# vniclas/VFM-Registration

Hardware: AMD Instinct MI355X
Metric: registrations/sec (20k<->200k pts, 384-D) (higher is better)
Workload: dtype fp6 (MX e2m3) coarse pass (scaled MFMA, fp32 scores + bounds from measured residuals) + int8 rescan (exact integer scores) + f32 refinement + f64 exact decision / f64 RANSAC

## Files before the change

### vfm-registration_amd/csrc/config.cpp

```cpp
#include "common.h"
#include "config.h"

#include <string.h>

#include <new>

struct vfm_config {
    VfmConfig c;
};

static const VfmConfig k_factory{};
static thread_local const VfmConfig* t_bound = nullptr;

const VfmConfig& vfm_cfg() { return t_bound ? *t_bound : k_factory; }

namespace {
struct Field {
    const char* name;
    int VfmConfig::*p;
};
const Field k_fields[] = {
    {"coarse_slices", &VfmConfig::force_slices},     {"match_stats", &VfmConfig::match_stats},
    {"i8_min_queries", &VfmConfig::i8_min_queries},  {"prep_grid", &VfmConfig::prep_grid},
    {"ransac_exact_only", &VfmConfig::ransac_exact_only}, {"ransac_fused", &VfmConfig::ransac_fused},
    {"coarse_qsets", &VfmConfig::coarse_qsets},      {"seed_units", &VfmConfig::seed_units},
    {"select_variant", &VfmConfig::select_variant},  {"mx6_t4", &VfmConfig::mx6_t4},
    {"mx6_tune", &VfmConfig::mx6_tune},
    {"mx6_ns3", &VfmConfig::mx6_ns3},                {"prep_form", &VfmConfig::prep_form},
    {"finish_short", &VfmConfig::finish_short},      {"rescan_rows", &VfmConfig::rescan_rows},
    {"half_noi8", &VfmConfig::half_noi8},            {"rescore_block", &VfmConfig::rescore_block},
    {"vit_preprocess_patch", &VfmConfig::vit_preprocess_patch}, {"vit_xcd", &VfmConfig::vit_xcd},
    {"vit_cfg_narrow", &VfmConfig::vit_cfg_narrow},  {"vit_cfg_wide", &VfmConfig::vit_cfg_wide},
    {"vit_wpw", &VfmConfig::vit_wpw},                {"vit_hot_a", &VfmConfig::vit_hot_a},
    {"vit_wide_tile", &VfmConfig::vit_wide_tile},    {"vit_lds_shape", &VfmConfig::vit_lds_shape},
    {"vit_att_lds_min", &VfmConfig::vit_att_lds_min}, {"vit_lds_min_wg", &VfmConfig::vit_lds_min_wg},
    {"vit_astat_min", &VfmConfig::vit_astat_min},    {"vit_astat_two", &VfmConfig::vit_astat_two},
    {"vit_astat_nw", &VfmConfig::vit_astat_nw},      {"vit_fused_qkv", &VfmConfig::vit_fused_qkv},
    {"vit_trace_fused", &VfmConfig::vit_trace_fused},  {"vit_fused_mlp", &VfmConfig::vit_fused_mlp},
    {"voxel_replay2", &VfmConfig::voxel_replay2},    {"voxel_one_launch", &VfmConfig::voxel_small},
    {"voxel_trace", &VfmConfig::voxel_trace},        {"voxel_grid_ppt", &VfmConfig::voxel_grid_ppt},
};

const char* const k_trace_buffer = "vit_trace_buffer";

void set_coarse_variant(VfmConfig& c, int v) {
    if (v == 60 || v == 61) { c.rescan_rows = v == 61 ? 1 : 0; return; }
    if (v == 50 || v == 51) { c.finish_short = v == 51 ? 1 : 0; return; }
    if (v >= 40 && v <= 44) { c.prep_form = v == 44 ? 4 : v == 43 ? 3 : v == 41 ? 1 : 0; return; }
    if (v == 32 || v == 33) { c.mx6_ns3 = v == 33 ? 1 : 0; return; }
    if (v == 30 || v == 31) { c.mx6_t4 = v == 30 ? 1 : 0; return; }
    c.seed_units = v == 7 ? 0 : 1;
    if (v == 7) v = 0;
    c.select_variant = v == 20 ? 1 : (v == 21 ? 2 : 0);
    if (v == 20 || v == 21) v = 0;
    c.coarse_qsets = v;
}
void set_voxel_small(VfmConfig& c, int on) {
    if (on == 2 || on == 3) c.voxel_replay2 = on == 3;
    else if (on >= 10 && on <= 10 + 64) c.voxel_grid_ppt = on - 10;
    else if (on == 100 || on == 101) c.voxel_trace = on - 100;
    else c.voxel_small = on;
}
}

VFM_EXPORT int vfm_config_create(vfm_config_t** out) {
    VFM_CHECK_ARG(out, "config_create: null pointer");
    *out = new (std::nothrow) vfm_config();
    if (!*out) return vfm_fail(VFM_EINVAL, "config_create: out of memory");
    return VFM_OK;
}
VFM_EXPORT int vfm_config_destroy(vfm_config_t* cfg) {
    if (cfg && t_bound == &cfg->c) t_bound = nullptr;
    delete cfg;
    return VFM_OK;
}
VFM_EXPORT int vfm_config_use(const vfm_config_t* cfg) {
    t_bound = cfg ? &cfg->c : nullptr;
    return VFM_OK;
}
VFM_EXPORT int vfm_config_set(vfm_config_t* cfg, const char* key, int64_t value) {
    VFM_CHECK_ARG(cfg && key, "config_set: null pointer");
    if ((!strcmp(key, "coarse_variant") && value == 42) || (!strcmp(key, "prep_form") && value == 2))
        return vfm_fail(VFM_EINVAL, "config_set: %s %lld (fp6 operand preparation by width) has been removed", key, (long long)value);
    if (!strcmp(key, "rescore_block") && value != 64 && value != 256)
        return vfm_fail(VFM_EINVAL, "config_set: rescore_block %lld (a workgroup of match_rescore_kernel owns 64 or 256 queries)", (long long)value);
    if (!strcmp(key, "coarse_variant")) { set_coarse_variant(cfg->c, (int)value); return VFM_OK; }
    if (!strcmp(key, "voxel_small")) { set_voxel_small(cfg->c, (int)value); return VFM_OK; }
    if (!strcmp(key, k_trace_buffer)) { cfg->c.vit_astat_dbg = reinterpret_cast<unsigned long long*>((uintptr_t)value); return VFM_OK; }
    for (const Field& f : k_fields)
        if (!strcmp(key, f.name)) {
            cfg->c.*(f.p) = (int)value;
            return VFM_OK;
        }
    return vfm_fail(VFM_EINVAL, "config_set: unknown key '%s'", key);
}
VFM_EXPORT int vfm_config_get(const vfm_config_t* cfg, const char* key, int64_t* value) {
    VFM_CHECK_ARG(key && value, "config_get: null pointer");
    const VfmConfig& c = cfg ? cfg->c : vfm_cfg();
    if (!strcmp(key, k_trace_buffer)) { *value = (int64_t)(uintptr_t)c.vit_astat_dbg; return VFM_OK; }
    for (const Field& f : k_fields)
        if (!strcmp(key, f.name)) {
            *value = c.*(f.p);
            return VFM_OK;
        }
    return vfm_fail(VFM_EINVAL, "config_get: unknown key '%s'", key);
}
```

### vfm-registration_amd/csrc/config.h

```cpp
#pragma once

struct VfmConfig {
    int force_slices = 0;
    int coarse_qsets = 0;
    int seed_units = 1;
    int select_variant = 0;
    int mx6_t4 = 1;
    int mx6_ns3 = 1;
    int prep_form = 3;
    int finish_short = 0;
    int half_noi8 = 1;
    int rescore_block = 0;
    int rescan_rows = 1;
    int mx6_tune = 0;
    int match_stats = 0;
    int i8_min_queries = 0;
    int prep_grid = -1;
    int ransac_exact_only = 0;
    int ransac_fused = 2;
    int vit_preprocess_patch = 1, vit_xcd = 1, vit_cfg_narrow = 108, vit_cfg_wide = 108, vit_wpw = 0, vit_hot_a = 0, vit_wide_tile = 0,
        vit_lds_shape = 23, vit_att_lds_min = 1, vit_lds_min_wg = 256, vit_astat_min = 0, vit_astat_two = 1, vit_astat_nw = 0,
        vit_trace_fused = 0,
        vit_fused_mlp = 0,
        vit_fused_qkv = 0;
    unsigned long long* vit_astat_dbg = nullptr;
    int voxel_replay2 = 1, voxel_small = 1, voxel_trace = 0, voxel_grid_ppt = 0;
};

const VfmConfig& vfm_cfg();
```

### vfm-registration_amd/csrc/match_internal.h

```cpp
#pragma once
#include "common.h"
#include "../../include/vfmreg_debug.h"

#include <type_traits>
#include <vector>

typedef _Float16 half8 __attribute__((ext_vector_type(8)));
typedef _Float16 half4 __attribute__((ext_vector_type(4)));
typedef float floatx16 __attribute__((ext_vector_type(16)));
typedef int intx4 __attribute__((ext_vector_type(4)));
typedef int intx8 __attribute__((ext_vector_type(8)));
typedef int intx16 __attribute__((ext_vector_type(16)));

#define GLOBAL_AS __attribute__((address_space(1)))
#define LDS_AS __attribute__((address_space(3)))

namespace vfmm {

constexpr int TILE_ROWS = 32;
constexpr int CHUNK_ROWS = 128;
constexpr int ROW_PAD = 256;
constexpr int QBLOCK = 256;
constexpr int ring_depth(int ksteps) { return ksteps <= 24 ? 6 : 4; }
constexpr int CAND_CAP_MAX = 2048;
// ... 681 lines not shown
        l.nqb = q2 ? (nq_tiles + 15) / 16 : npad / QBLOCK;
        l.nslices = choose_slices(l.nqb, nchunks);
        if (q2) inst = coarse_inst(CF_I8Q2, p.half ? d / 64 : d / 32, top2, !p.half, p.fused);
        else if (p.half) inst = coarse_inst(CF_I8, d / 64, 4, false, false);
        else inst = coarse_inst(CF_I8, d / 32, d <= 384 && (top2 || !t2) ? 4 : 2, top2, true);
    } else {
        const bool half = p.half, fuse = p.fused;
        const bool ns3 = half && fuse && d == 384 && cfg.mx6_ns3 && cfg.mx6_t4;
        l.nqb = ns3 ? (nq_tiles + 23) / 24 : (nq_tiles + 15) / 16;
        l.nslices = choose_slices(l.nqb, nchunks);
        if (half && cfg.force_slices == 0) {
            int s = (int)((1600 + l.nqb - 1) / l.nqb);
            const int smax = nchunks / 8 < 64 ? nchunks / 8 : 64;
            s = s > smax ? smax : s;
            s = s < 1 ? 1 : s;
            {
                const int cus = compute_units;
                int best = s;
                double best_fill = 0.0;
                for (int t = (s + 4 < smax ? s + 4 : smax); t >= 1 && t >= s - 12; --t) {
                    const long long wg = (long long)l.nqb * t, rounds = (wg + cus - 1) / cus;
                    const double fill = (double)wg / (double)(rounds * cus);
                    if (fill >= 0.975) {
                        best = t;
                        best_fill = 2.0;
                        break;
                    }
                    if (fill > best_fill) {
                        best_fill = fill;
                        best = t;
                    }
                }
                s = best;
            }
            l.nslices = s < 1 ? 1 : s;
        }
        while ((nchunks + l.nslices - 1) / l.nslices + 1 > MX6_LTAB && l.nslices < nchunks) ++l.nslices;
        if (fuse && (l.nqb > surv_slot_qblocks(npad) || l.nslices > surv_slot_slices(nchunks)))
            return vfm_fail(VFM_EINVAL, "search_coarse: %d x %d survivor slots exceed the workspace (n %d chunks %d)", l.nqb, l.nslices, npad, nchunks);
        const bool t8 = half && fuse && (d == 384 || d == 256) && !cfg.mx6_t4 && l.nslices <= nchunks / 2;
        l.tune = cfg.mx6_tune;
        const int ring = ns3 ? ((cfg.mx6_tune & 2) ? 5 : 4) : t8 ? 3 : 4;
        inst = coarse_inst(CF_MX6, half ? d / 128 : d / 64, fuse ? MX6_FUSE : top2 ? MX6_TOP2 : MX6_BEST, !half && !fuse, d / 64, ring, t8 ? 8 : 4, ns3 ? 3 : 2);
    }
    if (inst < 0) return vfm_fail(VFM_EINVAL, "search_coarse: no coarse kernel for d = %d, record kind %d", d, p.kind);
    l.inst = inst;
    l.seeded = l.nseed_pad != 0;
    l.block = coarse_inst_block(k_coarse_insts[inst]);
    l.lds = coarse_inst_lds(k_coarse_insts[inst]);
    return VFM_OK;
}
inline I8Bounds i8_bounds(const Prepared& Q, const Prepared& B, bool on, int top2 = 0) {
    return on ? I8Bounds{Q.err, Q.gstep, B.gstep, B.gerr, top2 == VFM_RECORDS_TOP2 ? 1 : 0} : I8Bounds{nullptr, nullptr, nullptr, nullptr, 0};
}
inline I8Bounds mx6_bounds(const Prepared& Q, const Prepared& B, int top2 = 0) { return I8Bounds{Q.err6, Q.gstep6, B.gstep6, B.gerr6, top2}; }
inline I8Bounds mx6_bounds_half(const Prepared& Q, const Prepared& B) { return I8Bounds{Q.err6h, Q.gstep6, B.gstep6, B.gerr6h, 0}; }
inline I8Bounds plan_bounds(const SearchPlan& p, const Prepared& Q, const Prepared& B) {
    if (p.bounds == BOUNDS_MX6_HALF) return mx6_bounds_half(Q, B);
    if (p.bounds == BOUNDS_MX6) return mx6_bounds(Q, B, p.top2 ? 1 : 0);
    return i8_bounds(Q, B, p.bounds == BOUNDS_I8, p.top2 ? 1 : 0);
}
CoarseArgs coarse_args(const Prepared& Q, const Prepared& B, const SearchWs& w, int64_t n, int64_t m);

struct PrepZero {
    uint4* a = nullptr;
    size_t na = 0;
    uint4* b = nullptr;
    size_t nb = 0;
};
inline PrepZero prep_zero(void* ws, int64_t n, int64_t m) {
    const SearchWs w = carve_search(ws, n, m);
    PrepZero z;
    z.a = reinterpret_cast<uint4*>(w.fb_count);
    z.na = search_zero_bytes(n, m) / 16;
    z.b = reinterpret_cast<uint4*>(w.cand_cnt);
    z.nb = (size_t)rows_padded(n) * sizeof(int) / 16;
    return z;
}
enum PrepInst : unsigned char {
    PREP_ROWS, PREP_CHUNK_BOTH, PREP_CHUNK_2, PREP_CHUNK_3, PREP_CHUNK_MX6,
    PREP_STREAM,
    PREP_ONCE = PREP_STREAM + 4,
    PREP_ONCE_NOI8 = PREP_ONCE + 8,
    PREP_MX6_ROWS_16 = PREP_ONCE_NOI8 + 4, PREP_MX6_ROWS_32, PREP_MX6_GROUP, PREP_INST_COUNT
};
inline const char* prep_inst_name(int inst) {
    static const char* const names[PREP_INST_COUNT] = {
        "prep_rows_kernel", "prep_chunk_kernel<true,2>", "prep_chunk_kernel<false,2>", "prep_chunk_kernel<false,3>", "prep_chunk_kernel<false,2,true,8>",
        "prep_stream_kernel<256,full>", "prep_stream_kernel<256,half>", "prep_stream_kernel<384,full>", "prep_stream_kernel<384,half>",
        "prep_once_kernel<256,full,short>", "prep_once_kernel<256,full,persist>", "prep_once_kernel<256,half,short>", "prep_once_kernel<256,half,persist>",
        "prep_once_kernel<384,full,short>", "prep_once_kernel<384,full,persist>", "prep_once_kernel<384,half,short>", "prep_once_kernel<384,half,persist>",
        "prep_once_kernel<256,half,short,noi8>", "prep_once_kernel<256,half,persist,noi8>", "prep_once_kernel<384,half,short,noi8>",
        "prep_once_kernel<384,half,persist,noi8>", "prep_mx6_rows_kernel<16>", "prep_mx6_rows_kernel<32>", "prep_mx6_group_kernel"};
    return names[inst];
}
enum PrepGridRule : unsigned char { PREP_GRID_ROWS, PREP_GRID_CU, PREP_GRID_2CU_STREAM, PREP_GRID_N };
enum PrepZeroAt : unsigned char { PREP_ZERO_NONE, PREP_ZERO_INSIDE, PREP_ZERO_BEHIND };
struct PrepLaunch {
    int inst;
    bool half6;
    int block, lds;
    int rule, n;
};
struct PrepPlan {
    bool f16 = false, i8 = false, fp6 = false, fp6_half = false;
    PrepLaunch launches[4] = {};
    int nlaunches = 0;
    int zero = PREP_ZERO_NONE;
};

inline int resolve_prepare(PrepPlan& p, int entry, int schedule, int d, int64_t rows1, int dtype1, int64_t rows2, int dtype2, bool zero) {
    p = PrepPlan{};
    const bool single = entry == VFM_PREP_ENTRY_PREPARE || entry == VFM_PREP_ENTRY_PERM;
    const bool gated = entry >= VFM_PREP_ENTRY_GATED && entry <= VFM_PREP_ENTRY_GATED_T;
    const bool scheduled = entry >= VFM_PREP_ENTRY_GATED_P && entry <= VFM_PREP_ENTRY_GATED_T;
    if (entry < VFM_PREP_ENTRY_PREPARE || entry > VFM_PREP_ENTRY_ONESHOT) return vfm_fail(VFM_EINVAL, "prepare: unknown entry %d", entry);
    if (!(rows1 > 0 && (single ? rows2 == 0 : rows2 > 0) && d % 128 == 0 && d >= 128 && d <= 768))
        return vfm_fail(VFM_EINVAL, "%s: d must be in {128,256,384,512,640,768}", entry == VFM_PREP_ENTRY_PREPARE ? "prepare" : "prepare2");
    if (entry == VFM_PREP_ENTRY_PERM && !i8_capable(d)) return vfm_fail(VFM_EINVAL, "prepare(perm): no int8 image for d = %d", d);
    VFM_CHECK_ARG((dtype1 == VFM_ROWS_F32 || dtype1 == VFM_ROWS_F16) && (dtype2 == VFM_ROWS_F32 || dtype2 == VFM_ROWS_F16) &&
                      (entry == VFM_PREP_ENTRY_GATED_T || (dtype1 == VFM_ROWS_F32 && dtype2 == VFM_ROWS_F32)), "prepare2: unknown row type");
    const int flags = VFM_PREPARE_MX6 | VFM_PREPARE_MX6_HALF | VFM_PREPARE_NO_I8;
    const int mode = schedule & ~flags;
    VFM_CHECK_ARG(scheduled ? mode >= VFM_PREPARE_DEFAULT && mode <= VFM_PREPARE_INTERLEAVED : schedule == 0, "prepare2: unknown schedule %d", schedule);
    const bool no_i8 = (schedule & VFM_PREPARE_NO_I8) != 0;
    const bool half6 = (schedule & VFM_PREPARE_MX6_HALF) != 0;
    const bool mx6 = half6 || (schedule & VFM_PREPARE_MX6) != 0;
    const bool any_f16 = dtype1 == VFM_ROWS_F16 || (rows2 > 0 && dtype2 == VFM_ROWS_F16);
    const int form = vfm_cfg().prep_form;
    const bool once = mx6 && mx6_width(d) && !any_f16 && (form == 3 || form == 4);
    if (no_i8) {
        VFM_CHECK_ARG(entry != VFM_PREP_ENTRY_GATED_T, "prepare2: VFM_PREPARE_NO_I8 is for fp32 rows (vfm_match_prepare2_gated_p / _z)");
        VFM_CHECK_ARG((schedule & VFM_PREPARE_MX6) && half6, "prepare2: VFM_PREPARE_NO_I8 needs VFM_PREPARE_MX6 | VFM_PREPARE_MX6_HALF (schedule %d)", schedule);
        VFM_CHECK_ARG(mx6_width(d), "prepare2: VFM_PREPARE_NO_I8 exists for d = 256 / 384, got %d", d);
    }
    const bool want_f16 = entry == VFM_PREP_ENTRY_PERM ? false : (gated || entry == VFM_PREP_ENTRY_ONESHOT) ? !use_i8(d, rows2, rows1, gated) : true;
    if (any_f16 && (want_f16 || !i8_capable(d)))
        return vfm_fail(VFM_EINVAL, "prepare: fp16 rows are taken by the gated int8 / fp6 searches (d in {256 .. 768}, more queries than the fp16 pass' limit)");
    if (no_i8 && !(once && rows2 > 0))
        return vfm_fail(VFM_EINVAL, "prepare: VFM_PREPARE_NO_I8 needs VFM_PREPARE_MX6_HALF, d = 256 / 384, fp32 rows of both operands and the "
                                    "one-read preparation (prep_form 3 / 4)");
    auto add = [&p](int inst, bool h6, int block, int lds, int rule, int n) { p.launches[p.nlaunches++] = PrepLaunch{inst, h6, block, lds, rule, n}; };
    auto add_rows = [&] { add(PREP_ROWS, false, 256, d * 64, PREP_GRID_ROWS, TILE_ROWS); };
    p.zero = !zero ? PREP_ZERO_NONE : once ? PREP_ZERO_INSIDE : PREP_ZERO_BEHIND;
    p.f16 = want_f16 || !i8_capable(d);
    if (!i8_capable(d)) {
        add_rows();
        return VFM_OK;
    }
    p.i8 = !no_i8;
    p.fp6 = mx6 && mx6_half_width(d);
    p.fp6_half = p.fp6 && half6;
    const int knob = mode == VFM_PREPARE_DEFAULT ? vfm_cfg().prep_grid : (mode == VFM_PREPARE_PERSISTENT ? 0 : -1);
    const int crule = knob > 0 ? PREP_GRID_N : (knob < 0 ? PREP_GRID_ROWS : PREP_GRID_CU), cn = knob > 0 ? knob : I8_GROUP;
    const int d384 = d == 384;
    if (once) {
        const int persist = form == 4, n = vfm_cfg().prep_grid;
        add(no_i8 ? PREP_ONCE_NOI8 + 2 * d384 + persist : PREP_ONCE + 4 * d384 + 2 * half6 + persist, half6, 256, 0,
            !persist ? PREP_GRID_ROWS : (n > 0 ? PREP_GRID_N : PREP_GRID_2CU_STREAM), persist && n > 0 ? n : I8_GROUP);
    } else if (mx6 && mx6_width(d) && form == 1 && !any_f16) {
        add(PREP_STREAM + 2 * d384 + half6, half6, 256, 0, PREP_GRID_ROWS, I8_GROUP);
    } else if (mx6 && mx6_width(d)) {
        add(PREP_CHUNK_MX6, half6, 512, I8_GROUP * (d * 3 + d / 8 + 16), crule, cn);
    } else if (want_f16 && d <= 384) {
        add(PREP_CHUNK_BOTH, false, 1024, I8_GROUP * d * 3, crule, cn);
        return VFM_OK;
    } else {
        add(d <= 512 ? PREP_CHUNK_2 : PREP_CHUNK_3, false, 1024, I8_GROUP * d, crule, cn);
    }
    if (want_f16) add_rows();
    if (p.fp6 && !mx6_width(d)) {
        add(d == 512 ? PREP_MX6_ROWS_16 : PREP_MX6_ROWS_32, half6, 256, (d == 512 ? 16 : 8) * d * 4, PREP_GRID_ROWS, d == 512 ? 16 : 8);
        add(PREP_MX6_GROUP, half6, 256, 0, PREP_GRID_ROWS, 4 * I8_GROUP);
    }
    return VFM_OK;
}

int do_prepare2(int entry, int schedule, Rows x1, int64_t rows1, void* prepared1, Rows x2, int64_t rows2, void* prepared2, int d,
                hipStream_t st, PrepZero zero = PrepZero{});
int do_prepare_perm(const float* x, int64_t rows, const int* perm, int d, void* prepared, hipStream_t st);
int launch_coarse(const CoarseLaunch& l, CoarseArgs& a, hipStream_t st);
typedef void (*CoarseKernel)(CoarseArgs);
int launch_coarse_kernel(CoarseKernel kernel, const char* what, const CoarseLaunch& l, const CoarseArgs& a, hipStream_t st);
int launch_coarse_f16(const CoarseLaunch& l, const CoarseArgs& a, hipStream_t st);
int launch_coarse_int8(const CoarseLaunch& l, const CoarseArgs& a, hipStream_t st);
int launch_coarse_mx6(const CoarseLaunch& l, const CoarseArgs& a, hipStream_t st);
int do_search_coarse(const void* qprep, int64_t n, const void* bprep, int64_t m, int d, void* ws, hipStream_t st,
                     bool bias_from_map_inv = false, bool inner_product = false, bool gated = false, int records = 0,
                     float gate = -__builtin_inff(), bool ws_clean = false);
int do_search_finish(Rows q, const void* qprep, int64_t n, Rows b, const void* bprep, int64_t m, int d,
                     int64_t* idx_out, float* sim_out, void* ws, hipStream_t st, bool gated = false,
                     float gate = -__builtin_inff(), int records = 0);
int launch_select_dense(const SearchWs& w, const CoarseArgs& a, const float* qinv, int64_t n, hipStream_t st);
int launch_i8_rescans(const SearchWs& w, const CoarseArgs& a, const Prepared& Q, const Prepared& B, int64_t n, int64_t m, int d,
                      bool use_bins, L2Terms l2, hipStream_t st);
int probe_half_select(const SearchPlan& plan, const void* qprep, int64_t n, const void* bprep, int64_t m, int d, void* ws, float gate, hipStream_t st);
int exact_ip_top1(const float* q, int64_t n, const float* b, int64_t m, int d, int64_t* idx_out, float* sim_out, void* ws,
                  hipStream_t st);
int launch_inv_norm(const float* x, int64_t rows, int d, float* inv_out, hipStream_t st);
int l2n_slices(int64_t nq, int64_t m);
size_t l2n_dir_bytes(int64_t nq, int64_t m, int d);
int l2n_search(const float* q, const int* qperm, int64_t nq, const float* b, int64_t m, int d, const unsigned* max_bits, int64_t* nn,
               double* d2, void* ws_dir, unsigned long long* evals, hipStream_t st);

}
```

### vfm-registration_amd/csrc/match_prep.hip

```cpp
#include "match_internal.h"

namespace vfmm {
namespace {

__device__ __forceinline__ void store_nt(uint4* dst, const uint4 t) {
    unsigned* o = reinterpret_cast<unsigned*>(dst);
    __builtin_nontemporal_store(t.x, o);
    __builtin_nontemporal_store(t.y, o + 1);
    __builtin_nontemporal_store(t.z, o + 2);
    __builtin_nontemporal_store(t.w, o + 3);
}

__global__ __launch_bounds__(256) void prep_rows_kernel(const float* __restrict__ x, int64_t rows, int d,
                                                        float* __restrict__ inv_out,
                                                        uint4* __restrict__ tiles, int tiles1,
                                                        const float* __restrict__ x2, int64_t rows2,
                                                        float* __restrict__ inv_out2, uint4* __restrict__ tiles2) {
    extern __shared__ __attribute__((aligned(16))) unsigned char smem[];
    int tile = blockIdx.x;
    if (tile >= tiles1) {
        tile -= tiles1;
        x = x2;
        rows = rows2;
        inv_out = inv_out2;
// ... 930 lines not shown
        unpack4(hh, nv);
        float e2 = 0.0f;
        *reinterpret_cast<unsigned*>(my8 + jr * RS8 + 4 * c) = quant4<false>(nv, qstep, inv_qstep, e2);
        if (c < 8 * nconv) {
            const int blk = c >> 3, k = (c & 7) >> 1, sub = c & 1;
            *reinterpret_cast<uint2*>(my16 + ((size_t)(k * nitems + jr * nconv + blk) * 16 + sub * 8)) = hh;
        }
        return e2;
    };
#pragma unroll
    for (int b = 0; b < 4; ++b) {
        __builtin_amdgcn_sched_barrier(0);
        float part[8];
#pragma unroll
        for (int j = 0; j < 8; ++j) part[j] = quant_chunk(hs0[8 * b + j], j, lane);
        if constexpr (PAIR && !NOI8) {
#pragma unroll
            for (int jp = 0; jp < 4; ++jp) {
                const float e2 = quant_chunk(hs1[4 * b + jp], 2 * jp + (lane >> 5), 64 + (lane & 31));
                part[2 * jp] = part[2 * jp] + (lo ? e2 : 0.0f);
                part[2 * jp + 1] = part[2 * jp + 1] + (lo ? 0.0f : e2);
            }
        }
        if constexpr (!NOI8) {
            const int64_t r = row0 + 8 * b + (lane >> 3);
            const float en = norm_up<true>(scatter8(part, lane), 1.0e-30f, false, r >= rows);
            if ((lane & 7) == 0) {
                o.err[r] = en;
                if (en > 0.0f) atomicMax(&emax_bits, __float_as_uint(en));
            }
        }
        __builtin_amdgcn_fence(__ATOMIC_RELEASE, "wavefront");
        __builtin_amdgcn_wave_barrier();
        __builtin_amdgcn_fence(__ATOMIC_ACQUIRE, "wavefront");
#ifndef VFM_POABL_NOST8
#pragma unroll
        for (int rd = 0; rd < (NOI8 ? 0 : (NU * 8 + 63) / 64); ++rd) {
            const int e = rd * 64 + lane, u = e >> 3, j = e & 7;
            if (e < NU * 8) {
                const uint4 tq = *reinterpret_cast<const uint4*>(my8 + j * RS8 + 16 * u);
                store_nt(tile8 + u * 32 + 8 * b + j, tq);
                if (!HALF && u < (NU >> 1)) store_nt(tile8h + u * 32 + 8 * b + j, tq);
            }
        }
#endif
        if (!NOI8 && o.rows8) {
#pragma unroll
            for (int rd = 0; rd < (NU * 8 + 63) / 64; ++rd) {
                const int e = rd * 64 + lane, j = e / NU, u = e - j * NU;
                if (e < NU * 8)
                    *reinterpret_cast<uint4*>(o.rows8 + (size_t)(row0 + 8 * b + j) * D + 16 * u) = *reinterpret_cast<const uint4*>(my8 + j * RS8 + 16 * u);
            }
        }
#ifndef VFM_POABL_NOMX6
#pragma unroll
        for (int item0 = 0; item0 < nitems; item0 += 64) {
            const int item = item0 + lane;
            if (item >= nitems) break;
            const int j = item / nconv, blk = item - j * nconv, p = 8 * b + j;
            Block6 vv;
#pragma unroll
            for (int k = 0; k < 4; ++k) vv.u[k] = *reinterpret_cast<const uint4*>(my16 + (size_t)(k * nitems + item) * 16);
            int ex;
            float e6;
            const intx6 codes = convert_block6(vv, ex, e6);
            store_codes<true>(tile6, blk >> 1, (blk & 1) * 32 + p, codes);
            l_sc[wave * 32 + p][blk] = (unsigned char)(ex + 127);
            l_e6[blk][wave * 32 + p] = e6;
        }
#endif
        __builtin_amdgcn_fence(__ATOMIC_RELEASE, "wavefront");
        __builtin_amdgcn_wave_barrier();
    }
    group_tail<D, HALF, NOI8>(o, grp, rows, tid, &l_sc[0][0], &l_e6[0][0], qstep, emax_bits, rmax_bits, e6max_bits, e6hmax_bits);
    if constexpr (!PERSIST) {
        break;
    } else {
        if (next >= groups) break;
        gidx = next;
    }
    }
}

template <int NBLK>
__global__ __launch_bounds__(256) void prep_mx6_rows_kernel(Rows x1, int64_t rows1, int64_t pad1, int d, PrepOut o1,
                                                            Rows x2, int64_t rows2, PrepOut o2, int64_t total) {
    constexpr int RPB = 256 / NBLK;
    const int blk = threadIdx.x % NBLK;
    int64_t g = (int64_t)blockIdx.x * RPB + threadIdx.x / NBLK;
    const bool beyond = g >= total;
    if (beyond) g = total - 1;
    const bool second = g >= pad1;
    const int64_t r = second ? g - pad1 : g;
    const int64_t rows = second ? rows2 : rows1;
    const PrepOut& o = second ? o2 : o1;
    const int nblk = d >> 5, nconv = o.mx6_half ? nblk >> 1 : nblk;
    const bool active = blk < nconv && !beyond;
    extern __shared__ __attribute__((aligned(16))) unsigned char mx6_smem[];
    float4* stage = reinterpret_cast<float4*>(mx6_smem);
    const int nf4 = d >> 2;
    const int64_t g0 = (int64_t)blockIdx.x * RPB;
    for (int idx = threadIdx.x; idx < RPB * nf4; idx += 256) {
        const int rr = idx / nf4, c4 = idx % nf4;
        const int64_t gg = g0 + rr;
        const bool sec = gg >= pad1;
        const int64_t r2 = sec ? gg - pad1 : gg;
        float4 t = make_float4(0.f, 0.f, 0.f, 0.f);
        if (gg < total && r2 < (sec ? rows2 : rows1)) {
            t = (sec ? x2 : x1).ld4_nt(r2 * (int64_t)d + 4 * c4);
        }
        const int bb = c4 >> 3, jj = c4 & 7;
        stage[rr * nf4 + bb * 8 + (jj ^ (bb & 7))] = t;
    }
    __syncthreads();
    Block6 v;
#pragma unroll
    for (int i = 0; i < 16; ++i) v.w[i] = 0u;
    if (active && r < rows) {
        const float iv = o.inv[r];
        const float4* mine = stage + (threadIdx.x / NBLK) * nf4 + blk * 8;
#pragma unroll
        for (int i = 0; i < 8; ++i) {
            const float4 t = mine[i ^ (blk & 7)];
            v.h[4 * i + 0] = (_Float16)(t.x * iv);
            v.h[4 * i + 1] = (_Float16)(t.y * iv);
            v.h[4 * i + 2] = (_Float16)(t.z * iv);
            v.h[4 * i + 3] = (_Float16)(t.w * iv);
        }
    }
    int ex;
    float e6;
    const intx6 codes = convert_block6(v, ex, e6);
    if (!active) e6 = 0.0f;
    float e6f = e6, e6hs = blk < (nblk >> 1) ? e6 : 0.0f;
#pragma unroll
    for (int off = NBLK / 2; off >= 1; off >>= 1) {
        e6f = e6f + __shfl_xor(e6f, off);
        e6hs = e6hs + __shfl_xor(e6hs, off);
    }
    if (blk == 0 && !beyond) {
        float e6n = sqrtf(e6f) * 1.000244140625f + (MX6_F16_ROUNDING + MX6_SLACK);
        float e6h = sqrtf(e6hs) * 1.000244140625f + (MX6_F16_ROUNDING + MX6_SLACK);
        if (!(e6n == e6n) || o.mx6_half) e6n = __builtin_inff();
        if (!(e6h == e6h)) e6h = __builtin_inff();
        if (r >= rows) e6n = e6h = 0.0f;
        o.err6[r] = e6n;
        o.err6h[r] = e6h;
    }
    if (active) {
        const int p = (int)(r & 31), s6 = blk >> 1, l6 = (blk & 1) * 32 + p, ks = d >> 6;
        unsigned char* tile = reinterpret_cast<unsigned char*>(o.tiles6) + (size_t)(r >> 5) * (size_t)mx6_tile_bytes(ks);
        store_codes<false>(tile, s6, l6, codes);
        tile[mx6_scale_at(ks, s6, l6)] = (unsigned char)(ex + 127);
    }
}

__global__ __launch_bounds__(256) void prep_mx6_group_kernel(PrepOut o1, int groups1, PrepOut o2, int groups) {
    const int gidx = blockIdx.x * 4 + (threadIdx.x >> 6);
    if (gidx >= groups) return;
    const bool second = gidx >= groups1;
    const PrepOut& o = second ? o2 : o1;
    const int grp = second ? gidx - groups1 : gidx;
    const int lane = lane_id();
    float m = fmaxf(o.err6[(int64_t)grp * I8_GROUP + lane], o.err6[(int64_t)grp * I8_GROUP + 64 + lane]);
    float mh = fmaxf(o.err6h[(int64_t)grp * I8_GROUP + lane], o.err6h[(int64_t)grp * I8_GROUP + 64 + lane]);
#pragma unroll
// ... 44 lines not shown
}

static unsigned prep_grid(const PrepLaunch& l, int64_t rows_pad, hipStream_t st) {
    if (l.rule == PREP_GRID_ROWS) return (unsigned)((rows_pad + l.n - 1) / l.n);
    int g = l.n;
    if (l.rule == PREP_GRID_CU) g = vfm_compute_units();
    if (l.rule == PREP_GRID_2CU_STREAM) {
        static thread_local hipStream_t last_st = nullptr;
        static thread_local int last_cus = 0;
        if (!last_cus || last_st != st) {
            int cus = vfm_compute_units();
            uint32_t mask[16] = {0};
            if (hipExtStreamGetCUMask(st, 16, mask) == hipSuccess) {
                int bits = 0;
                for (int i = 0; i < 16; ++i) bits += __builtin_popcount(mask[i]);
                if (bits > 0 && bits < cus) cus = bits;
            } else {
                (void)hipGetLastError();
            }
            last_st = st;
            last_cus = cus;
        }
        g = 2 * last_cus;
    }
    const int groups = (int)(rows_pad / I8_GROUP);
    return (unsigned)(g < groups ? g : groups);
}

static int launch_prepare(int entry, int schedule, Rows x1r, int64_t rows1, void* prepared1, Rows x2r, int64_t rows2, void* prepared2, int d,
                          const int* perm, hipStream_t st, PrepZero zero) {
    const size_t nz = zero.na + zero.nb;
    PrepPlan plan;
    static_assert(VFM_ROWS_F32 == 0 && VFM_ROWS_F16 == 1, "Rows::f16 carries the row type as passed");
    VFM_TRY(resolve_prepare(plan, entry, schedule, d, rows1, x1r.f16, rows2, x2r.f16, nz != 0));
    const Prepared p1 = carve_prepared(prepared1, rows1, d), p2 = rows2 ? carve_prepared(prepared2, rows2, d) : Prepared{};
    const float* x1 = static_cast<const float*>(x1r.p);
    const float* x2 = static_cast<const float*>(x2r.p);
    const int64_t pad1 = rows_padded(rows1), total = pad1 + (rows2 ? rows_padded(rows2) : 0);
    const int t1 = (int)(pad1 / TILE_ROWS), g1 = (int)(pad1 / I8_GROUP), groups = (int)(total / I8_GROUP);
    static unsigned long long attr_set = 0ull;
    if (i8_capable(d) && !attr_done(attr_set)) {
        VFM_CHECK_HIP(hipFuncSetAttribute(reinterpret_cast<const void*>(&prep_chunk_kernel<true, 2>),
                                          hipFuncAttributeMaxDynamicSharedMemorySize, I8_GROUP * 384 * 3));
        VFM_CHECK_HIP(hipFuncSetAttribute(reinterpret_cast<const void*>(&prep_chunk_kernel<false, 2>),
                                          hipFuncAttributeMaxDynamicSharedMemorySize, I8_GROUP * 512));
        VFM_CHECK_HIP(hipFuncSetAttribute(reinterpret_cast<const void*>(&prep_chunk_kernel<false, 3>),
                                          hipFuncAttributeMaxDynamicSharedMemorySize, I8_GROUP * 768));
        VFM_CHECK_HIP(hipFuncSetAttribute(reinterpret_cast<const void*>(&prep_chunk_kernel<false, 2, true, 8>),
                                          hipFuncAttributeMaxDynamicSharedMemorySize, I8_GROUP * (384 * 3 + 384 / 8 + 16)));
        attr_mark(attr_set);
    }
    for (int i = 0; i < plan.nlaunches; ++i) {
        const PrepLaunch& l = plan.launches[i];
        const dim3 grid(prep_grid(l, total, st)), block((unsigned)l.block);
        const PrepOut o1 = prep_out(p1, perm, l.half6), o2 = prep_out(p2, nullptr, l.half6);
        auto chunk = [&](auto kernel) { hipLaunchKernelGGL(kernel, grid, block, (size_t)l.lds, st, x1r, rows1, d, o1, g1, x2r, rows2, o2, groups); };
        auto stream = [&](auto kernel) { hipLaunchKernelGGL(kernel, grid, block, 0, st, x1, rows1, o1, g1, x2, rows2, o2, groups); };
        auto once = [&](auto kernel) { hipLaunchKernelGGL(kernel, grid, block, 0, st, x1, rows1, o1, g1, x2, rows2, o2, groups, zero); };
        auto mx6_rows = [&](auto kernel) { hipLaunchKernelGGL(kernel, grid, block, (size_t)l.lds, st, x1r, rows1, pad1, d, o1, x2r, rows2, o2, total); };
        switch (l.inst) {
            case PREP_ROWS:
                hipLaunchKernelGGL(prep_rows_kernel, grid, block, (size_t)l.lds, st, x1, rows1, d, p1.inv, p1.tiles, t1, x2, rows2, p2.inv, p2.tiles);
                break;
            case PREP_CHUNK_BOTH: chunk(prep_chunk_kernel<true, 2>); break;
            case PREP_CHUNK_2: chunk(prep_chunk_kernel<false, 2>); break;
            case PREP_CHUNK_3: chunk(prep_chunk_kernel<false, 3>); break;
            case PREP_CHUNK_MX6: chunk(prep_chunk_kernel<false, 2, true, 8>); break;
            case PREP_STREAM + 0: stream(prep_stream_kernel<256, false>); break;
            case PREP_STREAM + 1: stream(prep_stream_kernel<256, true>); break;
            case PREP_STREAM + 2: stream(prep_stream_kernel<384, false>); break;
            case PREP_STREAM + 3: stream(prep_stream_kernel<384, true>); break;
            case PREP_ONCE + 0: once(prep_once_kernel<256, false, false>); break;
            case PREP_ONCE + 1: once(prep_once_kernel<256, false, true>); break;
            case PREP_ONCE + 2: once(prep_once_kernel<256, true, false>); break;
            case PREP_ONCE + 3: once(prep_once_kernel<256, true, true>); break;
            case PREP_ONCE + 4: once(prep_once_kernel<384, false, false>); break;
            case PREP_ONCE + 5: once(prep_once_kernel<384, false, true>); break;
            case PREP_ONCE + 6: once(prep_once_kernel<384, true, false>); break;
            case PREP_ONCE + 7: once(prep_once_kernel<384, true, true>); break;
            case PREP_ONCE_NOI8 + 0: once(prep_once_kernel<256, true, false, true>); break;
            case PREP_ONCE_NOI8 + 1: once(prep_once_kernel<256, true, true, true>); break;
            case PREP_ONCE_NOI8 + 2: once(prep_once_kernel<384, true, false, true>); break;
            case PREP_ONCE_NOI8 + 3: once(prep_once_kernel<384, true, true, true>); break;
            case PREP_MX6_ROWS_16: mx6_rows(prep_mx6_rows_kernel<16>); break;
            case PREP_MX6_ROWS_32: mx6_rows(prep_mx6_rows_kernel<32>); break;
            case PREP_MX6_GROUP: hipLaunchKernelGGL(prep_mx6_group_kernel, grid, block, 0, st, o1, g1, o2, groups); break;
        }
        VFM_CHECK_LAUNCH(prep_inst_name(l.inst));
    }
    if (plan.zero == PREP_ZERO_BEHIND) {
        hipLaunchKernelGGL(prep_zero_kernel, dim3((unsigned)((nz + 255) / 256 < 1024 ? (nz + 255) / 256 : 1024)), dim3(256), 0, st, zero);
        VFM_CHECK_LAUNCH("prep_zero_kernel");
    }
    return VFM_OK;
}

int do_prepare2(int entry, int schedule, Rows x1, int64_t rows1, void* prepared1, Rows x2, int64_t rows2, void* prepared2, int d,
                hipStream_t st, PrepZero zero) {
    return launch_prepare(entry, schedule, x1, rows1, prepared1, x2, rows2, prepared2, d, nullptr, st, zero);
}

int do_prepare_perm(const float* x, int64_t rows, const int* perm, int d, void* prepared, hipStream_t st) {
    return launch_prepare(VFM_PREP_ENTRY_PERM, VFM_PREPARE_DEFAULT, x, rows, prepared, Rows(), 0, nullptr, d, perm, st, PrepZero{});
}

}

using namespace vfmm;

VFM_EXPORT int vfm_l2norm_rows_f32(float* x, int64_t n, int d, float* inv_out, vfm_stream_t stream) {
    VFM_CHECK_ARG(n >= 0 && d > 0 && d % 4 == 0 && d <= 1024, "l2norm: need d %% 4 == 0 and d <= 1024 (d=%d)", d);
    if (n == 0) return VFM_OK;
    hipLaunchKernelGGL(l2norm_rows_kernel, dim3((unsigned)((n + 3) / 4)), dim3(256), 0, (hipStream_t)stream, x, n, d,
                       inv_out);
    VFM_CHECK_LAUNCH("l2norm_rows_kernel");
    return VFM_OK;
}
```

### vfm-registration_amd/vfmreg/pipeline.py

```python
from __future__ import annotations

import contextlib
from typing import Optional

import numpy as np
import torch

from . import _lib, ops


class _ResultSet:
    def __init__(self, n: int, dev, qprep_bytes: int, bprep_bytes: int, sws_bytes: int):
        u8 = torch.uint8
        self.qprep = torch.empty(qprep_bytes, dtype=u8, device=dev)
        self.bprep = torch.empty(bprep_bytes, dtype=u8, device=dev)
        self.sws = torch.empty(sws_bytes, dtype=u8, device=dev)
        self.map_key: Optional[int] = None
        self.idx = torch.empty(n, dtype=torch.int64, device=dev)
        self.sim = torch.empty(n, dtype=torch.float32, device=dev)
        self.keep = torch.empty(n, dtype=torch.int64, device=dev)
        self.count = torch.zeros(1, dtype=torch.int64, device=dev)
        self.corres = torch.empty((n, 2), dtype=torch.int32, device=dev)
        self.T = torch.empty((4, 4), dtype=torch.float64, device=dev)
        self.fitness = torch.empty(1, dtype=torch.float64, device=dev)
# ... 42 lines not shown
        for _ in range(FEATURE_QUEUE_SKIP if TOUCH_STREAMS_AT_CREATION else 0):
            ph = torch.cuda.Stream(device=dev)
            with torch.cuda.stream(ph):
                torch.zeros(1, device=dev)
            _PLACEHOLDER_STREAMS.append(ph)
        fs = torch.cuda.Stream(device=dev, priority=int(priority))
        with torch.cuda.stream(fs):
            torch.zeros(1, device=dev)
        _FEATURE_STREAMS[key] = fs
    return _FEATURE_STREAMS[key]


class RegistrationPipeline:
    def __init__(self, n: int, m: int, d: int = 384, n_iter: int = 50000, min_cosine: float = 0.8,
                 max_corr_dist: float = 10000.0, seed: int = 42, device="cuda", overlap_ransac: bool = False,
                 overlap_prepare: bool = False, solve_streams: int = 1, gate: bool = True, coarse: str = "auto",
                 half_fused: Optional[bool] = None, prep_schedule: Optional[int] = None, private_streams: bool = False,
                 config: Optional["_lib.Config"] = None):
        lib = _lib.load()
        self.config = config
        self.n, self.m, self.d = n, m, d
        self.n_iter, self.min_cosine, self.max_corr_dist, self.seed = n_iter, min_cosine, max_corr_dist, seed
        self.device = torch.device(device)
        dev = self.device
        u8 = torch.uint8
        self.overlap = bool(overlap_ransac)
        self.overlap_prepare = bool(overlap_prepare)
        self.gate = bool(gate)
        if coarse not in ("auto", "int8-half", "int8", "int8-top2", "mx6", "mx6-top2", "mx6-pilot", "mx6-fused", "mx6-half", "fp16"):
            raise ValueError("coarse must be 'auto', 'int8-half', 'int8', 'int8-top2', 'mx6', 'mx6-top2', 'mx6-half' or 'fp16'")
        if coarse in ("int8-half", "mx6-half", "mx6-fused") and not gate:
            raise ValueError("the half-width pass (and the fused full-width one) need the gate")
        self.coarse = coarse
        self.use_i8 = coarse != "fp16"
        self.top2 = coarse == "int8-top2"
        self.mx6 = coarse in ("mx6", "mx6-top2", "mx6-pilot", "mx6-fused")
        self.mx6_fused = coarse == "mx6-fused"
        self.mx6_top2 = coarse == "mx6-top2"
        self.mx6_pilot = coarse == "mx6-pilot"
        self.half = coarse in ("int8-half", "mx6-half")
        self.mx6_half = coarse == "mx6-half"
        self._mx6_half_ok = coarse == "auto" and d in (256, 384, 512, 768) and n > 2048
        self._mx6_ok = self._mx6_half_ok and d in (256, 384)
        self._mx6_tried = False
        self._probe_due = coarse == "auto" and self.gate
        self._mx6_allowed = (self._mx6_ok, self._mx6_half_ok)
        self._fp6_off_by_reuse = False
        self._map_prepared = False
        self._half_kind = (3 if self.overlap else 4) if half_fused is None else (4 if half_fused else 3)
        self._mx6_half_kind = 7 if half_fused is False else 8
        self.last_rescans: Optional[int] = None
        self.last_probe: Optional[int] = None
        self._since_switch = 0
        self._pending = []
        self._slots = []
        self.n_solve = max(1, int(solve_streams)) if self.overlap else 0
        sizes = (lib.vfm_match_prepared_bytes(n, d), lib.vfm_match_prepared_bytes(m, d),
                 lib.vfm_match_search_workspace_bytes(n, m, d))
        self.sets = [_ResultSet(n, dev, *sizes) for _ in range(self.n_solve + 1)]
        shared_prep, shared_solve = (None, []) if (private_streams or not self.overlap) else _side_streams(dev, self.n_solve)
        self.solve_streams = shared_solve if shared_solve else [torch.cuda.Stream(device=dev) for _ in range(self.n_solve)]
        self.rws_list = [torch.empty(lib.vfm_ransac_workspace_bytes(n, n_iter), dtype=u8, device=dev)
                         for _ in range(max(1, self.n_solve))]
        self.rws = self.rws_list[0]
        self.ransac_stream = self.solve_streams[0] if self.overlap else None
        self.prep_stream = (shared_prep if shared_prep is not None else torch.cuda.Stream(device=dev)) if self.overlap else None
        self._step = 0
        self._prep_schedule = prep_schedule
        self._ws_clean = True
        self._noi8_shape = coarse == "auto" and self._resolves(8 | 0x200)
        self.last_prep_schedule: Optional[int] = None
        self.last_records: Optional[int] = None

    def _resolves(self, records: int) -> bool:
        try:
            with _lib.using(self.config) if self.config is not None else contextlib.nullcontext():
                _lib.search_plan(records, self.d, self.n, self.m)
            return True
        except RuntimeError:
            return False

    def _prepares_without_i8(self, records: int, probe: bool, f16_rows: bool) -> bool:
        return (records == 8 and self._noi8_shape and self._ws_clean and not probe and not f16_rows
                and _lib.policy("half_noi8") == 1 and _lib.policy("prep_form") in (3, 4))

    def prepare_map(self, b_desc: torch.Tensor) -> None:
        if self.config is None:
            return self._prepare_map(b_desc)
        with _lib.using(self.config):
            return self._prepare_map(b_desc)

    def _prepare_map(self, b_desc: torch.Tensor) -> None:
        lib = _lib.load()
        ops._chk(b_desc, torch.float32, "b_desc")
        if b_desc.shape != (self.m, self.d):
            raise ValueError("Invalid shape")
        if self.coarse in ("mx6", "mx6-top2", "mx6-pilot", "mx6-fused", "mx6-half"):
            raise ValueError("the fp6 modes prepare map and scan together in every registration: no prepare_map()")
        self._mx6_ok = self._mx6_half_ok = False
        self.mx6 = self.mx6_half = False
        self._map_prepared = True
        main = torch.cuda.current_stream()
        for r in self.sets:
            if r.done is not None:
                main.wait_event(r.done)
            _lib.check(lib.vfm_match_prepare(b_desc.data_ptr(), self.m, self.d, r.bprep.data_ptr(), main.cuda_stream),
                       "prepare(map)")
            r.map_key = b_desc.data_ptr()

    HALF_LIMIT = 24.0
    RESCAN_LIMIT = 128.0
    MX6_UP = 128.0
    MX6_DOWN = 400.0
    PILOT_UP = 1.0e9
    TOP2_LIMIT = 40
    REPROBE = 256

    def _poll_feedback(self) -> None:
        while self._pending and self._pending[0][0].query():
            _, slot, records = self._pending.pop(0)
            if records == "probe":
                self.last_probe = int(slot.item())
                self._slots.append(slot)
                if self.coarse == "auto" and self.use_i8 and not self.half and self.last_probe <= self.HALF_LIMIT * self.n:
                    self.half, self.top2, self.mx6 = True, False, False
                    self.mx6_half = self._mx6_half_ok
                    self._since_switch = 0
                continue
            self.last_rescans = int(slot.item())
            self._slots.append(slot)
            if self.coarse != "auto" or not self.use_i8 or records != self._records():
                continue
            if self.half:
                if self.last_rescans > self.HALF_LIMIT * self.n:
                    if self.mx6_half and self.last_probe is not None and self.last_probe <= self.HALF_LIMIT * self.n:
                        self.mx6_half = False
                    else:
                        self.half = False
                    self._since_switch = 0
            elif self.mx6:
                if self.last_rescans > self.MX6_DOWN * self.n:
                    self.mx6, self._mx6_tried = False, True
                    self._since_switch = 0
                elif not self.mx6_pilot and self.last_rescans > self.PILOT_UP * self.n:
                    self.mx6_pilot = True
                    self._since_switch = 0
            elif not self.top2 and self.last_rescans > self.RESCAN_LIMIT * self.n:
                self.top2 = True
                self._since_switch = 0
            elif not self.top2 and self._mx6_ok and not self._mx6_tried and self.last_rescans <= self.MX6_UP * self.n:
                self.mx6 = True
                self._since_switch = 0
            elif self.top2 and self.last_rescans > self.TOP2_LIMIT * self.n:
                self.use_i8 = False
                self._since_switch = 0

    def _records(self) -> int:
        if self.mx6:
            if self.mx6_fused:
                return 10
            return 6 if self.mx6_top2 else (9 if self.mx6_pilot else 5)
        if self.half and self.mx6_half:
            return self._mx6_half_kind
        return self._half_kind if self.half else (1 if self.top2 else 0)

    def synchronize(self) -> None:
        for s in self.solve_streams:
# ... 316 lines not shown
```

Baseline: 2221.

## Add one-pass fp6 preparation kernel for the no-int8 path

Adds prep_onepass_kernel, which normalizes fp32 rows, computes inverse norms and residual norms, converts to fp6 blocks and writes scales in one read of the input. It uses cross-lane permlane swaps and DPP reductions in place of LDS round trips. When the no-int8 schedule is requested and prep_form was not set explicitly, it becomes the default (form 5). The goal is to cut memory traffic and synchronisation in the preparation step, at the cost of heavier register use and a new, intricate lane-mapping code path.

```diff
diff --git a/vfm-registration_amd/csrc/config.cpp b/vfm-registration_amd/csrc/config.cpp
--- a/vfm-registration_amd/csrc/config.cpp
+++ b/vfm-registration_amd/csrc/config.cpp
@@ -46,7 +46,7 @@
 void set_coarse_variant(VfmConfig& c, int v) {
     if (v == 60 || v == 61) { c.rescan_rows = v == 61 ? 1 : 0; return; }
     if (v == 50 || v == 51) { c.finish_short = v == 51 ? 1 : 0; return; }
-    if (v >= 40 && v <= 44) { c.prep_form = v == 44 ? 4 : v == 43 ? 3 : v == 41 ? 1 : 0; return; }
+    if (v >= 40 && v <= 45) { c.prep_form_set = 1; c.prep_form = v == 45 ? 5 : v == 44 ? 4 : v == 43 ? 3 : v == 41 ? 1 : 0; return; }
     if (v == 32 || v == 33) { c.mx6_ns3 = v == 33 ? 1 : 0; return; }
     if (v == 30 || v == 31) { c.mx6_t4 = v == 30 ? 1 : 0; return; }
     c.seed_units = v == 7 ? 0 : 1;
@@ -87,6 +87,7 @@
     if (!strcmp(key, "coarse_variant")) { set_coarse_variant(cfg->c, (int)value); return VFM_OK; }
     if (!strcmp(key, "voxel_small")) { set_voxel_small(cfg->c, (int)value); return VFM_OK; }
     if (!strcmp(key, k_trace_buffer)) { cfg->c.vit_astat_dbg = reinterpret_cast<unsigned long long*>((uintptr_t)value); return VFM_OK; }
+    if (!strcmp(key, "prep_form")) cfg->c.prep_form_set = 1;
     for (const Field& f : k_fields)
         if (!strcmp(key, f.name)) {
             cfg->c.*(f.p) = (int)value;
diff --git a/vfm-registration_amd/csrc/config.h b/vfm-registration_amd/csrc/config.h
--- a/vfm-registration_amd/csrc/config.h
+++ b/vfm-registration_amd/csrc/config.h
@@ -8,6 +8,7 @@
     int mx6_t4 = 1;
     int mx6_ns3 = 1;
     int prep_form = 3;
+    int prep_form_set = 0;
     int finish_short = 0;
     int half_noi8 = 1;
     int rescore_block = 0;
diff --git a/vfm-registration_amd/csrc/match_internal.h b/vfm-registration_amd/csrc/match_internal.h
--- a/vfm-registration_amd/csrc/match_internal.h
+++ b/vfm-registration_amd/csrc/match_internal.h
@@ -787,7 +787,8 @@
     PREP_STREAM,
     PREP_ONCE = PREP_STREAM + 4,
     PREP_ONCE_NOI8 = PREP_ONCE + 8,
-    PREP_MX6_ROWS_16 = PREP_ONCE_NOI8 + 4, PREP_MX6_ROWS_32, PREP_MX6_GROUP, PREP_INST_COUNT
+    PREP_ONEPASS = PREP_ONCE_NOI8 + 4,
+    PREP_MX6_ROWS_16 = PREP_ONEPASS + 2, PREP_MX6_ROWS_32, PREP_MX6_GROUP, PREP_INST_COUNT
 };
 inline const char* prep_inst_name(int inst) {
     static const char* const names[PREP_INST_COUNT] = {
@@ -796,7 +797,7 @@
         "prep_once_kernel<256,full,short>", "prep_once_kernel<256,full,persist>", "prep_once_kernel<256,half,short>", "prep_once_kernel<256,half,persist>",
         "prep_once_kernel<384,full,short>", "prep_once_kernel<384,full,persist>", "prep_once_kernel<384,half,short>", "prep_once_kernel<384,half,persist>",
         "prep_once_kernel<256,half,short,noi8>", "prep_once_kernel<256,half,persist,noi8>", "prep_once_kernel<384,half,short,noi8>",
-        "prep_once_kernel<384,half,persist,noi8>", "prep_mx6_rows_kernel<16>", "prep_mx6_rows_kernel<32>", "prep_mx6_group_kernel"};
+        "prep_once_kernel<384,half,persist,noi8>", "prep_onepass_kernel<256>", "prep_onepass_kernel<384>", "prep_mx6_rows_kernel<16>", "prep_mx6_rows_kernel<32>", "prep_mx6_group_kernel"};
     return names[inst];
 }
 enum PrepGridRule : unsigned char { PREP_GRID_ROWS, PREP_GRID_CU, PREP_GRID_2CU_STREAM, PREP_GRID_N };
@@ -832,8 +833,8 @@
     const bool half6 = (schedule & VFM_PREPARE_MX6_HALF) != 0;
     const bool mx6 = half6 || (schedule & VFM_PREPARE_MX6) != 0;
     const bool any_f16 = dtype1 == VFM_ROWS_F16 || (rows2 > 0 && dtype2 == VFM_ROWS_F16);
-    const int form = vfm_cfg().prep_form;
-    const bool once = mx6 && mx6_width(d) && !any_f16 && (form == 3 || form == 4);
+    const int form = !vfm_cfg().prep_form_set && (schedule & VFM_PREPARE_NO_I8) ? 5 : vfm_cfg().prep_form;
+    const bool once = mx6 && mx6_width(d) && !any_f16 && (form == 3 || form == 4 || form == 5);
     if (no_i8) {
         VFM_CHECK_ARG(entry != VFM_PREP_ENTRY_GATED_T, "prepare2: VFM_PREPARE_NO_I8 is for fp32 rows (vfm_match_prepare2_gated_p / _z)");
         VFM_CHECK_ARG((schedule & VFM_PREPARE_MX6) && half6, "prepare2: VFM_PREPARE_NO_I8 needs VFM_PREPARE_MX6 | VFM_PREPARE_MX6_HALF (schedule %d)", schedule);
@@ -844,7 +845,7 @@
         return vfm_fail(VFM_EINVAL, "prepare: fp16 rows are taken by the gated int8 / fp6 searches (d in {256 .. 768}, more queries than the fp16 pass' limit)");
     if (no_i8 && !(once && rows2 > 0))
         return vfm_fail(VFM_EINVAL, "prepare: VFM_PREPARE_NO_I8 needs VFM_PREPARE_MX6_HALF, d = 256 / 384, fp32 rows of both operands and the "
-                                    "one-read preparation (prep_form 3 / 4)");
+                                    "one-read preparation (prep_form 3 / 4 / 5)");
     auto add = [&p](int inst, bool h6, int block, int lds, int rule, int n) { p.launches[p.nlaunches++] = PrepLaunch{inst, h6, block, lds, rule, n}; };
     auto add_rows = [&] { add(PREP_ROWS, false, 256, d * 64, PREP_GRID_ROWS, TILE_ROWS); };
     p.zero = !zero ? PREP_ZERO_NONE : once ? PREP_ZERO_INSIDE : PREP_ZERO_BEHIND;
@@ -861,7 +862,8 @@
     const int d384 = d == 384;
     if (once) {
         const int persist = form == 4, n = vfm_cfg().prep_grid;
-        add(no_i8 ? PREP_ONCE_NOI8 + 2 * d384 + persist : PREP_ONCE + 4 * d384 + 2 * half6 + persist, half6, 256, 0,
+        if (no_i8 && form == 5) add(PREP_ONEPASS + d384, true, 256, 0, PREP_GRID_ROWS, I8_GROUP);
+        else add(no_i8 ? PREP_ONCE_NOI8 + 2 * d384 + persist : PREP_ONCE + 4 * d384 + 2 * half6 + persist, half6, 256, 0,
             !persist ? PREP_GRID_ROWS : (n > 0 ? PREP_GRID_N : PREP_GRID_2CU_STREAM), persist && n > 0 ? n : I8_GROUP);
     } else if (mx6 && mx6_width(d) && form == 1 && !any_f16) {
         add(PREP_STREAM + 2 * d384 + half6, half6, 256, 0, PREP_GRID_ROWS, I8_GROUP);
diff --git a/vfm-registration_amd/csrc/match_prep.hip b/vfm-registration_amd/csrc/match_prep.hip
--- a/vfm-registration_amd/csrc/match_prep.hip
+++ b/vfm-registration_amd/csrc/match_prep.hip
@@ -1036,6 +1036,193 @@
     }
 }
 
+template <int CTRL>
+__device__ __forceinline__ float dpp_mov(float x) {
+    return __int_as_float(__builtin_amdgcn_update_dpp(0, __float_as_int(x), CTRL, 0xf, 0xf, true));
+}
+__device__ __forceinline__ float dpp_xor8(float x) { return dpp_mov<0x128>(x); }
+__device__ __forceinline__ float dpp_xor4(float x) { return dpp_mov<0x1b>(dpp_mov<0x141>(x)); }
+__device__ __forceinline__ float dpp_xor2(float x) { return dpp_mov<0x4e>(x); }
+__device__ __forceinline__ float dpp_xor1(float x) { return dpp_mov<0xb1>(x); }
+
+__device__ __forceinline__ float scatter8_dpp(const float* p, int lane) {
+    const bool b5 = (lane & 32) != 0, b4 = (lane & 16) != 0, b3 = (lane & 8) != 0;
+    float q4[4], q2[2];
+#pragma unroll
+    for (int j = 0; j < 4; ++j) {
+        const auto sw = __builtin_amdgcn_permlane32_swap(__float_as_uint(p[j]), __float_as_uint(p[j + 4]), false, false);
+        const float e = __uint_as_float((unsigned)sw[0]), o = __uint_as_float((unsigned)sw[1]);
+        q4[j] = (b5 ? o : e) + (b5 ? e : o);
+    }
+#pragma unroll
+    for (int j = 0; j < 2; ++j) {
+        const auto sw = __builtin_amdgcn_permlane16_swap(__float_as_uint(q4[j]), __float_as_uint(q4[j + 2]), false, false);
+        const float e = __uint_as_float((unsigned)sw[0]), o = __uint_as_float((unsigned)sw[1]);
+        q2[j] = (b4 ? o : e) + (b4 ? e : o);
+    }
+    float q1 = (b3 ? q2[1] : q2[0]) + dpp_xor8(b3 ? q2[0] : q2[1]);
+    q1 = q1 + dpp_xor4(q1);
+    q1 = q1 + dpp_xor2(q1);
+    q1 = q1 + dpp_xor1(q1);
+    return q1;
+}
+
+template <bool B>
+struct PrepGuard {
+    static constexpr bool value = B;
+};
+
+template <int D>
+__global__ __launch_bounds__(256, 2) void prep_onepass_kernel(const float* __restrict__ x1, int64_t rows1, PrepOut o1, int groups1,
+                                                              const float* __restrict__ x2, int64_t rows2, PrepOut o2, int groups, PrepZero z) {
+    constexpr bool PAIR = D > 256;
+    constexpr int NBLK = D >> 5;
+    constexpr int nconv = NBLK >> 1;
+    constexpr int nitems = 8 * nconv;
+    static_assert(D == 256 || D == 384, "a lane owns one chunk (d = 256) or one and a half (d = 384) of a row");
+    static_assert(nitems <= 64, "a batch's items are converted by one wave at once");
+    __shared__ __attribute__((aligned(16))) unsigned char l_h16[4][4 * nitems * 16];
+    __shared__ float l_e6[NBLK][I8_GROUP];
+    __shared__ unsigned char l_sc[I8_GROUP][16];
+    __shared__ unsigned emax_bits, rmax_bits, e6max_bits, e6hmax_bits;
+    const int tid = threadIdx.x, lane = lane_id();
+    const int wave = __builtin_amdgcn_readfirstlane(tid >> 6);
+    if (z.na + z.nb) {
+        const size_t nz = z.na + z.nb;
+        for (size_t i = (size_t)blockIdx.x * 256 + threadIdx.x; i < nz; i += (size_t)gridDim.x * 256)
+            *(i < z.na ? z.a + i : z.b + (i - z.na)) = make_uint4(0u, 0u, 0u, 0u);
+    }
+    const int gidx = blockIdx.x;
+    const bool second = gidx >= groups1;
+    const int grp = second ? gidx - groups1 : gidx;
+    const float* x = second ? x2 : x1;
+    const int64_t rows = second ? rows2 : rows1;
+    const PrepOut& o = second ? o2 : o1;
+    const int64_t row0 = (int64_t)grp * I8_GROUP + wave * 32;
+    const bool lo = lane < 32;
+    if (tid == 0) {
+        emax_bits = 0u;
+        rmax_bits = 0u;
+        e6max_bits = 0u;
+        e6hmax_bits = 0u;
+    }
+    __syncthreads();
+    unsigned char* my16 = l_h16[wave];
+    unsigned char* tile6 = reinterpret_cast<unsigned char*>(o.tiles6) + ((size_t)grp * 4 + wave) * (size_t)mx6_tile_bytes(D >> 6);
+    auto tile = [&](auto G) __attribute__((always_inline)) {
+        constexpr bool GUARD = decltype(G)::value;
+        float4 v0[8];
+        float4 vp[PAIR ? 4 : 1];
+        auto load4 = [&](int64_t r, int c) __attribute__((always_inline)) {
+            float4 t = make_float4(0.f, 0.f, 0.f, 0.f);
+            if (!GUARD || r < rows) {
+                const float* pc = x + r * (int64_t)D + 4 * c;
+                t.x = __builtin_nontemporal_load(pc);
+                t.y = __builtin_nontemporal_load(pc + 1);
+                t.z = __builtin_nontemporal_load(pc + 2);
+                t.w = __builtin_nontemporal_load(pc + 3);
+            }
+            return t;
+        };
+        auto load_row = [&](int b, int j) __attribute__((always_inline)) { v0[j] = load4(row0 + 8 * b + j, lane); };
+        auto load_pair = [&](int b, int jp) __attribute__((always_inline)) { vp[jp] = load4(row0 + 8 * b + 2 * jp + (lane >> 5), 64 + (lane & 31)); };
+        auto lo_lo = [&](float a, float b) __attribute__((always_inline)) {
+            const auto sw = __builtin_amdgcn_permlane32_swap(__float_as_uint(a), __float_as_uint(b), false, false);
+            return __uint_as_float((unsigned)sw[0]);
+        };
+        auto hi_to_lo = [&](float a) __attribute__((always_inline)) {
+            const auto sw = __builtin_amdgcn_permlane32_swap(__float_as_uint(a), __float_as_uint(a), false, false);
+            return __uint_as_float((unsigned)sw[1]);
+        };
+#pragma unroll
+        for (int j = 0; j < 8; ++j) load_row(0, j);
+        if constexpr (PAIR) {
+#pragma unroll
+            for (int jp = 0; jp < 4; ++jp) load_pair(0, jp);
+        }
+        unsigned rmax = 0u;
+#pragma unroll
+        for (int b = 0; b < 4; ++b) {
+            __builtin_amdgcn_sched_barrier(0);
+            float part[8];
+#pragma unroll
+            for (int j = 0; j < 8; ++j) part[j] = fold4(0.0f, v0[j]);
+            if constexpr (PAIR) {
+#pragma unroll
+                for (int jp = 0; jp < 4; ++jp) {
+                    const float s = fold4(lo_lo(part[2 * jp], part[2 * jp + 1]), vp[jp]);
+                    const float sb = hi_to_lo(s);
+                    part[2 * jp] = lo ? s : part[2 * jp];
+                    part[2 * jp + 1] = lo ? sb : part[2 * jp + 1];
+                }
+            }
+            const float my_inv = inv_norm_from_sumsq(scatter8_dpp(part, lane));
+            if ((lane & 7) == 0) o.inv[row0 + 8 * b + (lane >> 3)] = my_inv;
+            float rpart[8], ivs[8];
+            uint2 hs[8];
+#pragma unroll
+            for (int j = 0; j < 8; ++j) {
+                const float iv = __uint_as_float(__builtin_amdgcn_readlane(__float_as_uint(my_inv), 8 * j));
+                ivs[j] = iv;
+                const float nv[4] = {v0[j].x * iv, v0[j].y * iv, v0[j].z * iv, v0[j].w * iv};
+                const float ss = nv[0] * nv[0] + nv[1] * nv[1] + nv[2] * nv[2] + nv[3] * nv[3];
+                float r2 = 0.0f;
+                r2 = r2 + ((8 * lane >= D) ? ss : 0.0f);
+                const half4 h = round_half4(nv);
+                __builtin_memcpy(&hs[j], &h, 8);
+                asm volatile("" : "+v"(r2), "+v"(hs[j].x), "+v"(hs[j].y));
+                rpart[j] = r2;
+                if (b < 3) load_row(b + 1, j);
+            }
+            if constexpr (PAIR) {
+#pragma unroll
+                for (int jp = 0; jp < 4; ++jp) {
+                    const float iv = lo ? ivs[2 * jp] : ivs[2 * jp + 1];
+                    const float nv[4] = {vp[jp].x * iv, vp[jp].y * iv, vp[jp].z * iv, vp[jp].w * iv};
+                    float ss = nv[0] * nv[0] + nv[1] * nv[1] + nv[2] * nv[2] + nv[3] * nv[3];
+                    asm volatile("" : "+v"(ss));
+                    const float ssb = hi_to_lo(ss);
+                    rpart[2 * jp] = rpart[2 * jp] + (lo ? ss : 0.0f);
+                    rpart[2 * jp + 1] = rpart[2 * jp + 1] + (lo ? ssb : 0.0f);
+                    if (b < 3) load_pair(b + 1, jp);
+                }
+            }
+            {
+                const int64_t r = row0 + 8 * b + (lane >> 3);
+                const float rn = norm_up(scatter8_dpp(rpart, lane), 1.0e-30f, false, r >= rows);
+                if ((lane & 7) == 0) o.rest[r] = rn;
+                if (rn > 0.0f) rmax = max(rmax, __float_as_uint(rn));
+            }
+            if (lane < 8 * nconv) {
+                const int blk = lane >> 3, k = (lane & 7) >> 1, sub = lane & 1;
+#pragma unroll
+                for (int j = 0; j < 8; ++j) *reinterpret_cast<uint2*>(my16 + ((size_t)(k * nitems + j * nconv + blk) * 16 + sub * 8)) = hs[j];
+            }
+            __builtin_amdgcn_fence(__ATOMIC_RELEASE, "wavefront");
+            __builtin_amdgcn_wave_barrier();
+            __builtin_amdgcn_fence(__ATOMIC_ACQUIRE, "wavefront");
+            if (lane < nitems) {
+                const int j = lane / nconv, blk = lane - j * nconv, p = 8 * b + j;
+                Block6 vv;
+#pragma unroll
+                for (int k = 0; k < 4; ++k) vv.u[k] = *reinterpret_cast<const uint4*>(my16 + (size_t)(k * nitems + lane) * 16);
+                int ex;
+                float e6;
+                const intx6 codes = convert_block6(vv, ex, e6);
+                store_codes<true>(tile6, blk >> 1, (blk & 1) * 32 + p, codes);
+                l_sc[wave * 32 + p][blk] = (unsigned char)(ex + 127);
+                l_e6[blk][wave * 32 + p] = e6;
+            }
+            __builtin_amdgcn_fence(__ATOMIC_RELEASE, "wavefront");
+            __builtin_amdgcn_wave_barrier();
+        }
+        if ((lane & 7) == 0 && rmax) atomicMax(&rmax_bits, rmax);
+    };
+    if (row0 + 32 <= rows) tile(PrepGuard<false>{});
+    else tile(PrepGuard<true>{});
+    group_tail<D, true, true>(o, grp, rows, tid, &l_sc[0][0], &l_e6[0][0], 1.0f, emax_bits, rmax_bits, e6max_bits, e6hmax_bits);
+}
+
 template <int NBLK>
 __global__ __launch_bounds__(256) void prep_mx6_rows_kernel(Rows x1, int64_t rows1, int64_t pad1, int d, PrepOut o1,
                                                             Rows x2, int64_t rows2, PrepOut o2, int64_t total) {
@@ -1246,6 +1433,8 @@
             case PREP_ONCE_NOI8 + 1: once(prep_once_kernel<256, true, true, true>); break;
             case PREP_ONCE_NOI8 + 2: once(prep_once_kernel<384, true, false, true>); break;
             case PREP_ONCE_NOI8 + 3: once(prep_once_kernel<384, true, true, true>); break;
+            case PREP_ONEPASS + 0: once(prep_onepass_kernel<256>); break;
+            case PREP_ONEPASS + 1: once(prep_onepass_kernel<384>); break;
             case PREP_MX6_ROWS_16: mx6_rows(prep_mx6_rows_kernel<16>); break;
             case PREP_MX6_ROWS_32: mx6_rows(prep_mx6_rows_kernel<32>); break;
             case PREP_MX6_GROUP: hipLaunchKernelGGL(prep_mx6_group_kernel, grid, block, 0, st, o1, g1, o2, groups); break;
diff --git a/vfm-registration_amd/vfmreg/pipeline.py b/vfm-registration_amd/vfmreg/pipeline.py
--- a/vfm-registration_amd/vfmreg/pipeline.py
+++ b/vfm-registration_amd/vfmreg/pipeline.py
@@ -148,7 +148,7 @@
 
     def _prepares_without_i8(self, records: int, probe: bool, f16_rows: bool) -> bool:
         return (records == 8 and self._noi8_shape and self._ws_clean and not probe and not f16_rows
-                and _lib.policy("half_noi8") == 1 and _lib.policy("prep_form") in (3, 4))
+                and _lib.policy("half_noi8") == 1 and _lib.policy("prep_form") in (3, 4, 5))
 
     def prepare_map(self, b_desc: torch.Tensor) -> None:
         if self.config is None:
```

Result: no change. 2237, median of 6 (+0.7%).
